# alexkeroro86/SampleNeRFRO

Hardware: AMD Instinct MI355X
Metric: rays/sec (train step) (higher is better)
Workload: dtype f16x3/fp32-acc

## Files before the change

### samplenerfro_amd/csrc/mlp.hip

```cpp
#include "common.h"
#include "nerfmlp_layout.h"
#include "mfma_ops.h"
#include "bkgd_layout.h"
#include "so3_layout.h"

#include <stdlib.h>
#include <type_traits>
#include <vector>
#include <stdio.h>

namespace rnerf {


#define GLOBAL_AS __attribute__((address_space(1)))
#define LDS_AS __attribute__((address_space(3)))

struct MfmaLayer { int dense, ks, nt, kind; };
__host__ __device__ constexpr MfmaLayer mfma_layer(int l) {
  constexpr MfmaLayer t[10] = {{0, 4, 8, 0},  {1, 16, 8, 1}, {2, 16, 8, 1}, {3, 16, 8, 1}, {4, 16, 8, 1},
                               {5, 20, 8, 2}, {6, 16, 8, 1}, {7, 16, 8, 1}, {9, 16, 8, 1}, {10, 18, 4, 3}};
  return t[l];
}
__host__ __device__ constexpr int layer_blocks_before(int l) {
  int o = 0;
// ... 117 lines not shown
    for (int j = 0; j < 8; ++j) {
      const int f = in_feature(l, s, h, j);
      w[j] = f < 0 ? 0.f : params[nerf_koff(d) + f * out_dim + n_out] * PP::WSCALE;
      if constexpr (PP::F16) { if (!(fabsf(w[j]) <= 65504.f)) ((float*)(packed + PP::STREAM_BYTES))[AUX_FLAG] = 1.0f; }
    }
    uint32_t hi[4], lo[4];
    for (int p = 0; p < 4; ++p) split2<F16>(w[2 * p], w[2 * p + 1], hi[p], lo[p]);
    if constexpr (PP::F8X) {
      f8x_mode();
      float wl[8], ws[8];
      for (int p = 0; p < 4; ++p) {
        float ha, hb;
        unpack2<true>(hi[p], ha, hb);
        wl[2 * p] = w[2 * p] - ha; wl[2 * p + 1] = w[2 * p + 1] - hb;
        ws[2 * p] = w[2 * p] * (1.0f / F8X_LO_SCALE); ws[2 * p + 1] = w[2 * p + 1] * (1.0f / F8X_LO_SCALE);
      }
      lo[0] = f8_pair<true>(f8_pair<false>(0u, wl[0], wl[1]), wl[2], wl[3]); lo[1] = f8_pair<true>(f8_pair<false>(0u, wl[4], wl[5]), wl[6], wl[7]);
      lo[2] = f8_pair<true>(f8_pair<false>(0u, ws[0], ws[1]), ws[2], ws[3]); lo[3] = f8_pair<true>(f8_pair<false>(0u, ws[4], ws[5]), ws[6], ws[7]);
    }
    uint4* dst = (uint4*)(packed + (size_t)blk * PP::NP * 1024);
    dst[lane] = make_uint4(hi[0], hi[1], hi[2], hi[3]);
    if constexpr (PP::F8X) { uint2* d2 = (uint2*)(dst + 64); d2[lane] = make_uint2(lo[0], lo[1]); d2[64 + lane] = make_uint2(lo[2], lo[3]); }
    else if (PP::NP == 2) dst[64 + lane] = make_uint4(lo[0], lo[1], lo[2], lo[3]);
  }
  float* aux = (float*)(packed + PP::STREAM_BYTES);
  if (gid < AUX_FLAG) {
    float v = 0.f;
    if (gid < AUX_WSIG) {
      const int l = gid >> 8, n = gid & 255, d = mfma_layer(l).dense;
      v = n < nerf_dense(d).out ? params[nerf_boff(d) + n] : 0.f;
    } else if (gid < AUX_BSIG) v = params[nerf_koff(8) + (gid - AUX_WSIG)];
    else if (gid == AUX_BSIG) v = params[nerf_boff(8)];
    else if (gid >= AUX_WRGB && gid < AUX_BRGB) { const int c = (gid - AUX_WRGB) / 128, n = (gid - AUX_WRGB) % 128; v = params[nerf_koff(11) + n * 3 + c]; }
    else if (gid >= AUX_BRGB && gid < AUX_BRGB + 3) v = params[nerf_boff(11) + (gid - AUX_BRGB)];
    aux[gid] = v;
  }
}

__device__ __forceinline__ void glds16(const char* gsrc, unsigned lds_off) {
  unsigned keep;
  asm volatile("s_mov_b32 %0, m0\n\ts_mov_b32 m0, %2\n\ts_nop 0\n\tglobal_load_lds_dwordx4 %1, off\n\ts_mov_b32 m0, %0"
               : "=&s"(keep) : "v"(gsrc), "s"(lds_off) : "memory");
}
__device__ __forceinline__ void glds16_nt(const char* gsrc, unsigned lds_off) {
  unsigned keep;
  asm volatile("s_mov_b32 %0, m0\n\ts_mov_b32 m0, %2\n\ts_nop 0\n\tglobal_load_lds_dwordx4 %1, off nt\n\ts_mov_b32 m0, %0"
               : "=&s"(keep) : "v"(gsrc), "s"(lds_off) : "memory");
}
__device__ __forceinline__ void glds16_nt_s(const char* sbase, unsigned voff, unsigned lds_off) {
  unsigned keep;
  asm volatile("s_mov_b32 %0, m0\n\ts_mov_b32 m0, %3\n\ts_nop 0\n\tglobal_load_lds_dwordx4 %1, %2 nt\n\ts_mov_b32 m0, %0"
               : "=&s"(keep) : "v"(voff), "s"(sbase), "s"(lds_off) : "memory");
}
__device__ __forceinline__ void slab_wait_dma() { __builtin_amdgcn_s_waitcnt(0x0F70); asm volatile("" ::: "memory"); }

template <int BYTES>
__device__ __forceinline__ void issue_slab(const char* __restrict__ gsrc, unsigned lds_off, int wave, int lane) {
  constexpr int PER_WAVE = BYTES / 4;
  constexpr int N = PER_WAVE / 1024;
  static_assert(N >= 1 && N * 4096 == BYTES, "slab must be a multiple of 4 KiB");
#pragma unroll
  for (int c = 0; c < N; ++c)
    glds16(gsrc + wave * PER_WAVE + c * 1024 + lane * 16,
           __builtin_amdgcn_readfirstlane(lds_off + wave * PER_WAVE + c * 1024));
}

__device__ __forceinline__ uint32_t pk_maxu(uint32_t a, uint32_t b) {
  uint32_t r;
  asm("v_pk_max_u16 %0, %1, %2" : "=v"(r) : "v"(a), "v"(b));
  return r;
}
__device__ __forceinline__ uint32_t pk_min1(uint32_t w) {
  uint32_t r;
  asm("v_pk_min_u16 %0, %1, %2" : "=v"(r) : "v"(w), "v"(0x00010001u));
  return r;
}

typedef float f32x4v __attribute__((ext_vector_type(4)));
__device__ __forceinline__ float4 gload4(const float* p) {
  const f32x4v v = *(const __attribute__((address_space(1))) f32x4v*)p;
  return make_float4(v.x, v.y, v.z, v.w);
}

template <bool ONE_> struct KOpsT { static constexpr bool ONE = ONE_; uint4 h0, l0, h1, l1; };
typedef KOpsT<false> KOps;

constexpr int RELU_FLOOR = 0, NO_FLOOR = (int)0x80000000u;
__device__ __forceinline__ float relu_keep(float x, int floor_bits) {
  const int b = __builtin_bit_cast(int, x);
  return __builtin_bit_cast(float, b > floor_bits ? b : floor_bits);
}

typedef unsigned int u32x4_t __attribute__((ext_vector_type(4)));
__device__ __forceinline__ void stream_store(uint4* p, const uint4 v) {
  u32x4_t t = {v.x, v.y, v.z, v.w};
  __builtin_nontemporal_store(t, (u32x4_t*)p);
}
__device__ __forceinline__ uint4 stream_load(const uint4* p) {
  const u32x4_t t = __builtin_nontemporal_load((const u32x4_t*)p);
  return make_uint4(t.x, t.y, t.z, t.w);
}
typedef unsigned int u32x2_t __attribute__((ext_vector_type(2)));
__device__ __forceinline__ void stream_store8(uint2* p, const uint2 v) {
  u32x2_t t = {v.x, v.y};
  __builtin_nontemporal_store(t, (u32x2_t*)p);
}

// ... 414 lines not shown
      float f[2][8];
#pragma unroll
      for (int mt = 0; mt < (ONE ? 1 : 2); ++mt)
#pragma unroll
        for (int j = 0; j < 8; ++j) {
          const int q = 8 * s + j;
          if (q < nsin) {
            const int d = q / 3, c = q % 3;
            const float x = c == 0 ? v[mt].x : (c == 1 ? v[mt].y : v[mt].z);
            f[mt][j] = pe_sin(fadd(fmul(x, (float)(1 << d)), phase));
          } else if (q == nsin) f[mt][j] = h ? v[mt].z : v[mt].x;
          else if (q == nsin + 1) f[mt][j] = h ? 0.f : v[mt].y;
          else f[mt][j] = 0.f;
        }
      KOps o;
      split8<PREC>(f[0], o.h0, o.l0);
      if constexpr (ONE) { o.h1 = o.h0; o.l1 = o.l0; } else split8<PREC>(f[1], o.h1, o.l1);
      return o;
    };

    auto prev_ops = [&](int s, const float* __restrict__ bias, int floor_v) -> KOps {
      const float4 b0 = *(const float4*)(bias + 16 * s + 4 * h), b1 = *(const float4*)(bias + 16 * s + 8 + 4 * h);
      const float bb[8] = {b0.x, b0.y, b0.z, b0.w, b1.x, b1.y, b1.z, b1.w};
      float r1[8] = {0.f, 0.f, 0.f, 0.f, 0.f, 0.f, 0.f, 0.f};
      if constexpr (!ONE) {
        const float4 u0 = st1[((s >> 1) * 4 + 2 * (s & 1)) * 64], u1 = st1[((s >> 1) * 4 + 2 * (s & 1) + 1) * 64];
        r1[0] = u0.x; r1[1] = u0.y; r1[2] = u0.z; r1[3] = u0.w; r1[4] = u1.x; r1[5] = u1.y; r1[6] = u1.z; r1[7] = u1.w;
      }
      float x0[8], x1[8];
#pragma unroll
      for (int j = 0; j < 8; ++j) {
        x0[j] = relu_keep(fmaf(prev0[s >> 1][8 * (s & 1) + j], INV_SCALE, bb[j]), floor_v);
        x1[j] = relu_keep(fmaf(r1[j], INV_SCALE, bb[j]), floor_v);
      }
      KOps o;
      split8<PREC>(x0, o.h0, o.l0);
      if constexpr (ONE) { o.h1 = o.h0; o.l1 = o.l0; } else split8<PREC>(x1, o.h1, o.l1);
      return o;
    };

    auto load_bias8 = [&](int s, const float* __restrict__ bias, float (&b)[8]) {
      const float4 b0 = *(const float4*)(bias + 16 * s + 4 * h), b1 = *(const float4*)(bias + 16 * s + 8 + 4 * h);
      b[0] = b0.x; b[1] = b0.y; b[2] = b0.z; b[3] = b0.w; b[4] = b1.x; b[5] = b1.y; b[6] = b1.z; b[7] = b1.w;
    };
    auto load_state8 = [&](int s, float (&v)[8]) {
      if constexpr (ONE) return;
      const float4 u0 = st1[((s >> 1) * 4 + 2 * (s & 1)) * 64], u1 = st1[((s >> 1) * 4 + 2 * (s & 1) + 1) * 64];
      v[0] = u0.x; v[1] = u0.y; v[2] = u0.z; v[3] = u0.w; v[4] = u1.x; v[5] = u1.y; v[6] = u1.z; v[7] = u1.w;
    };
    NoWork nowork;

#define SLAB_PREFETCH(DO_NEXT)                                                                                       \
  do { if (DO_NEXT) { issue_slab<SLAB>(packed + off, (unsigned)((buf ^ 1) * SLAB), wave, lane); off += SLAB; } } while (0)
#define SLAB_DONE() do { slab_wait_dma(); __syncthreads(); buf ^= 1; } while (0)

    float sig0 = 0.f, sig1 = 0.f;

    KOps cur;
    {
      cur = enc_ops(pd, 0, 30);
      SeamWork<PREC, TRAIN != 0, ONE> seam(acc0, acc1, prev0, st1);
      seam.cv.floor_v = RELU_FLOOR;
      load_bias8(0, auxt + AUX_BIAS, seam.cv.b);
      load_bias8(0, auxt + AUX_ZERO, seam.cv.ws);
#define RNERF_PE_KSTEP(S, FIRST_, SAVE_)                                                                             \
      {                                                                                                              \
        if (SAVE_) save_ops(SAVE_PE + S, cur);                                                                       \
        watch(cur, true);          \
        SLAB_PREFETCH(true);    \
        if constexpr (S < 3) {                                                                                       \
          EncWork<PREC, S + 1, 30, ONE> ew(pd, h);                                                                        \
          kstep_mfma<PREC, 8, 0, FIRST_>(acc0, acc1, cur, smem + buf * SLAB, lane, ew);                              \
          cur = ew.result();                                                                                         \
        } else {                                                                                                     \
          kstep_mfma<PREC, 8, 0, false>(acc0, acc1, cur, smem + buf * SLAB, lane, seam);                             \
        }                                                                                                            \
        SLAB_DONE();                                                                                                 \
      }
      RNERF_PE_KSTEP(0, true, true) RNERF_PE_KSTEP(1, false, true) RNERF_PE_KSTEP(2, false, true) RNERF_PE_KSTEP(3, false, true)
      seam.finish();
      cur = seam.cv.result();
    }

    float bnext[8], wnext[8];
    load_bias8(1, auxt + AUX_BIAS, bnext);
    load_bias8(1, auxt + AUX_ZERO, wnext);

#pragma unroll 1
    for (int l = 1; l <= 8; ++l) {
      const float* __restrict__ bias = auxt + AUX_BIAS + 256 * (l - 1);
      SeamWork<PREC, TRAIN != 0, ONE> seam(acc0, acc1, prev0, st1);
      seam.cv.floor_v = l == 8 ? NO_FLOOR : RELU_FLOOR;
      const float* __restrict__ wseam = auxt + (l == 7 ? AUX_WSIG : AUX_ZERO);
      const float* __restrict__ wsel = auxt + (l == 8 ? AUX_WSIG : AUX_ZERO);
#define RNERF_KSTEP(S)                                                                                              \
      {                                                                                                              \
        save_ops(SAVE_L1 + 16 * (l - 1) + S, cur);                                                                   \
        watch(cur, false);                                                                                           \
        if constexpr (TRAIN != 0 && S == 0) save_mask(l - 1, 0, nz_nibbles(cur.h0), nz_nibbles(cur.h1));                  \
        if constexpr (S == 13) { load_bias8(0, bias + 256, seam.cv.b); load_bias8(0, wseam, seam.cv.ws); }           \
        float bnn[8], wnn[8];                                                                                        \
        if constexpr (S + 2 < 16) { load_bias8(S + 2, bias, bnn); load_bias8(S + 2, wsel, wnn); }    \
        else if constexpr (S == 14) { load_bias8(1, bias + 256, bnn); load_bias8(1, wseam, wnn); }    \
        auto dma = [&]() { SLAB_PREFETCH(true); };                                                                   \
        if constexpr (S + 1 < 16) {                                                                                  \
          PrevConv<PREC, S + 1, TRAIN != 0, true, ONE> cv(prev0[(S + 1) >> 1]);                                           \
          cv.floor_v = RELU_FLOOR;                                                                                        \
          _Pragma("unroll") for (int j = 0; j < 8; ++j) { cv.b[j] = bnext[j]; cv.ws[j] = wnext[j]; }                 \
          load_state8(S + 1, cv.v1);                                                                                 \
          kstep_mfma<PREC, 8, 0, S == 0, PrevConv<PREC, S + 1, TRAIN != 0, true, ONE>, decltype(dma)>(acc0, acc1, cur, smem + buf * SLAB, lane, cv, dma); \
          cur = cv.result();                                                                                         \
          sig0 += cv.sg0; sig1 += cv.sg1;                                                                            \
          save_mask(l - 1, S + 1, cv.nz[0], cv.nz[1]);                                                               \
        } else {                                                                                                     \
           \
           \
          kstep_mfma<PREC, 8, 0, false, SeamWork<PREC, TRAIN != 0, ONE>, decltype(dma)>(acc0, acc1, cur, smem + buf * SLAB, lane, seam, dma); \
        }                                                                                                            \
        if constexpr (S + 2 <= 16) { _Pragma("unroll") for (int j = 0; j < 8; ++j) { bnext[j] = bnn[j]; wnext[j] = wnn[j]; } } \
        SLAB_DONE();                                                                                                 \
      }
      RNERF_KSTEP(0) RNERF_KSTEP(1) RNERF_KSTEP(2) RNERF_KSTEP(3) RNERF_KSTEP(4) RNERF_KSTEP(5) RNERF_KSTEP(6) RNERF_KSTEP(7)
      RNERF_KSTEP(8) RNERF_KSTEP(9) RNERF_KSTEP(10) RNERF_KSTEP(11) RNERF_KSTEP(12) RNERF_KSTEP(13) RNERF_KSTEP(14) RNERF_KSTEP(15)
#undef RNERF_KSTEP
      if (l == 5) {
        asm volatile("" : "+v"(pd[0].x), "+v"(pd[0].y), "+v"(pd[0].z), "+v"(pd[1].x), "+v"(pd[1].y), "+v"(pd[1].z));
        cur = enc_ops(pd, 0, 30);
        RNERF_PE_KSTEP(0, false, false) RNERF_PE_KSTEP(1, false, false) RNERF_PE_KSTEP(2, false, false) RNERF_PE_KSTEP(3, false, false)
      }
      seam.finish();
      cur = seam.cv.result();
      sig0 += seam.cv.sg0; sig1 += seam.cv.sg1;
    }

    {
      const float* __restrict__ bias = auxt + AUX_BIAS + 256 * 8;
      KOps c0 = cur;
      KOps c1 = prev_ops(1, bias, NO_FLOOR);
      float bA[8], bB[8];
      load_bias8(2, bias, bA);
      load_bias8(3, bias, bB);
#define RNERF_VSLAB(SL)                                                                                              \
      {                                                                                                              \
        save_ops(SAVE_L1 + 16 * 8 + 2 * SL, c0);                                                                     \
        save_ops(SAVE_L1 + 16 * 8 + 2 * SL + 1, c1);                                                                 \
        watch(c0, true); watch(c1, true);                                                                            \
        SLAB_PREFETCH(true);                                                                                         \
        if constexpr (SL + 1 < 8) {                                                                                  \
          float bA2[8], bB2[8];                                                                                      \
          if constexpr (SL + 2 < 8) { load_bias8(2 * SL + 4, bias, bA2); load_bias8(2 * SL + 5, bias, bB2); }        \
          PrevConv<PREC, 2 * SL + 2, false, false, ONE> cvA(prev0[SL + 1]);                                                      \
          PrevConv<PREC, 2 * SL + 3, false, false, ONE> cvB(prev0[SL + 1]);                                                      \
          cvA.floor_v = NO_FLOOR; cvB.floor_v = NO_FLOOR;                                                                \
          _Pragma("unroll") for (int j = 0; j < 8; ++j) { cvA.b[j] = bA[j]; cvB.b[j] = bB[j]; }                      \
          load_state8(2 * SL + 2, cvA.v1);                                                                           \
          load_state8(2 * SL + 3, cvB.v1);                                                                           \
          PairOfPairs<decltype(cvA)> wA(cvA);                                                                        \
          PairOfPairs<decltype(cvB)> wB(cvB);                                                                        \
          kstep_mfma<PREC, 4, 0, SL == 0>(acc0, acc1, c0, smem + buf * SLAB, lane, wA);                              \
          kstep_mfma<PREC, 4, 1, false>(acc0, acc1, c1, smem + buf * SLAB, lane, wB);                                \
          c0 = cvA.result(); c1 = cvB.result();                                                                      \
          if constexpr (SL + 2 < 8) { _Pragma("unroll") for (int j = 0; j < 8; ++j) { bA[j] = bA2[j]; bB[j] = bB2[j]; } } \
        } else {                                                                                                     \
          const KOps n0 = enc_ops(dr, 0, 12), n1 = enc_ops(dr, 1, 12);                                               \
          kstep_mfma<PREC, 4, 0, false>(acc0, acc1, c0, smem + buf * SLAB, lane, nowork);                            \
          kstep_mfma<PREC, 4, 1, false>(acc0, acc1, c1, smem + buf * SLAB, lane, nowork);                            \
          c0 = n0; c1 = n1;                                                                                          \
        }                                                                                                            \
        SLAB_DONE();                                                                                                 \
      }
      RNERF_VSLAB(0) RNERF_VSLAB(1) RNERF_VSLAB(2) RNERF_VSLAB(3) RNERF_VSLAB(4) RNERF_VSLAB(5) RNERF_VSLAB(6) RNERF_VSLAB(7)
#undef RNERF_VSLAB
      save_ops(SAVE_VIEW, c0);
      save_ops(SAVE_VIEW + 1, c1);
      watch(c0, true); watch(c1, true);
      next_tile = tileq != nullptr ? __builtin_amdgcn_readfirstlane(__hip_atomic_load(tileq + 1 + blockIdx.x, __ATOMIC_RELAXED, __HIP_MEMORY_SCOPE_AGENT))
                                   : find_next(tile + (int)gridDim.x);
      const bool has_next_tile = next_tile < n_tiles;
      if (has_next_tile) off = 0;
      SLAB_PREFETCH(has_next_tile);
      kstep_mfma<PREC, 4, 0, false>(acc0, acc1, c0, smem + buf * SLAB, lane, nowork);
      kstep_mfma<PREC, 4, 1, false>(acc0, acc1, c1, smem + buf * SLAB, lane, nowork);
      SLAB_DONE();
    }

    {
      const float* __restrict__ hw = auxt + 4 * h;
      auto head_load = [&](int t, float4 (&W)[16]) {
#pragma unroll
        for (int g = 0; g < 4; ++g) {
          const int n = 32 * t + 8 * g;
          W[4 * g] = gload4(hw + AUX_BIAS + 256 * 9 + n);
          W[4 * g + 1] = gload4(hw + AUX_WRGB + n); W[4 * g + 2] = gload4(hw + AUX_WRGB + 128 + n); W[4 * g + 3] = gload4(hw + AUX_WRGB + 256 + n);
        }
      };
      float p0[3] = {0.f, 0.f, 0.f}, p1[3] = {0.f, 0.f, 0.f};
      float4 Wc[16];
      head_load(0, Wc);
#pragma unroll
      for (int t = 0; t < 4; ++t) {
        float4 Wn[16];
        if (t + 1 < 4) head_load(t + 1, Wn);
        RNERF_PIN();
        float rv0[16], rv1[16];
#pragma unroll
        for (int g = 0; g < 4; ++g) {
          const float4 bb = Wc[4 * g], wr = Wc[4 * g + 1], wg = Wc[4 * g + 2], wb = Wc[4 * g + 3];
          const float bv[4] = {bb.x, bb.y, bb.z, bb.w}, wrv[4] = {wr.x, wr.y, wr.z, wr.w}, wgv[4] = {wg.x, wg.y, wg.z, wg.w}, wbv[4] = {wb.x, wb.y, wb.z, wb.w};
#pragma unroll
          for (int i = 0; i < 4; ++i) {
            const float v0 = relu_keep(fmaf(acc0[t][4 * g + i], INV_SCALE, bv[i]), RELU_FLOOR);
            p0[0] = fmaf(v0, wrv[i], p0[0]); p0[1] = fmaf(v0, wgv[i], p0[1]); p0[2] = fmaf(v0, wbv[i], p0[2]);
            rv0[4 * g + i] = v0;
            if constexpr (!ONE) {
              const float v1 = relu_keep(fmaf(acc1[t][4 * g + i], INV_SCALE, bv[i]), RELU_FLOOR);
              p1[0] = fmaf(v1, wrv[i], p1[0]); p1[1] = fmaf(v1, wgv[i], p1[1]); p1[2] = fmaf(v1, wbv[i], p1[2]);
              rv1[4 * g + i] = v1;
            } else rv1[4 * g + i] = v0;
          }
        }
        if (t + 1 < 4) {
#pragma unroll
          for (int q = 0; q < 16; ++q) Wc[q] = Wn[q];
        }
        if constexpr (TRAIN != 0) {
#pragma unroll
          for (int half = 0; half < 2; ++half) {
            KOps o;
            float a0[8], a1[8];
#pragma unroll
            for (int j = 0; j < 8; ++j) { a0[j] = rv0[8 * half + j]; a1[j] = rv1[8 * half + j]; }
            if constexpr (TRAIN >= 2) { split8<PREC>(a0, o.h0, o.l0); split8<PREC>(a1, o.h1, o.l1); }
            else {
              o.h0 = make_uint4(pack2<PP::F16>(a0[0], a0[1]), pack2<PP::F16>(a0[2], a0[3]), pack2<PP::F16>(a0[4], a0[5]), pack2<PP::F16>(a0[6], a0[7]));
              o.h1 = make_uint4(pack2<PP::F16>(a1[0], a1[1]), pack2<PP::F16>(a1[2], a1[3]), pack2<PP::F16>(a1[4], a1[5]), pack2<PP::F16>(a1[6], a1[7]));
            }
// ... 20 lines not shown
      }
      if constexpr (PP::F16 && !PP::F8X) {
        if (auxt[AUX_FLAG] != 0.f) { const float qn = __builtin_nanf(""); p0[0] = p0[1] = p0[2] = qn; p1[0] = p1[1] = p1[2] = qn; sig0 = qn; sig1 = qn; }
      }
      if (h == 0) {
        if constexpr (REDO) {
          if (row_ok[0] && __builtin_isnan(out_raw[row[0]].x)) out_raw[row[0]] = make_float4(p0[0], p0[1], p0[2], sig0);
          if (row_ok[1] && __builtin_isnan(out_raw[row[1]].x)) out_raw[row[1]] = make_float4(p1[0], p1[1], p1[2], sig1);
        } else {
          if (row_ok[0]) out_raw[row[0]] = make_float4(p0[0], p0[1], p0[2], sig0);
          if (row_ok[1]) out_raw[row[1]] = make_float4(p1[0], p1[1], p1[2], sig1);
        }
      }
    }
#undef RNERF_PE_KSTEP
#undef SLAB_PREFETCH
#undef SLAB_DONE
    tile = next_tile;
  }
}

constexpr int DY_L9 = 144, DY_HEADS = 152, DY_SLOTS = 153;
constexpr int DGRAD_PASSES = 22;
constexpr int kBwdF16OnePass = 3;
constexpr int kBwdBlocks = 8 * 8 + 8 * 16 * 8;

__host__ __device__ constexpr int bwd_dense(int i) { return i == 0 ? 10 : (i == 1 ? 9 : 9 - i); }
__host__ __device__ constexpr int bwd_blocks_before(int i) { return i == 0 ? 0 : 64 + (i - 1) * 128; }

template <int PREC>
__global__ void nerfmlp_pack_bwd_kernel(const float* __restrict__ params, char* __restrict__ packed) {
  using PP = Prec<PREC>;
  const int gid = blockIdx.x * blockDim.x + threadIdx.x;
  if (gid >= kBwdBlocks * 64) return;
  const int blk = gid >> 6, lane = gid & 63;
  int i = 0;
  while (i < 8 && blk >= bwd_blocks_before(i + 1)) ++i;
  const int rel = blk - bwd_blocks_before(i);
  const int s = rel / 8, kt = rel % 8;
  const int d = bwd_dense(i), out_dim = nerf_dense(d).out;
  const int kf = 32 * kt + (lane & 31), h = lane >> 5;
  float w[8];
  for (int j = 0; j < 8; ++j) {
    const int n = prev_feature(s, h, j);
    w[j] = n < out_dim ? params[nerf_koff(d) + kf * out_dim + n] * PP::WSCALE : 0.f;
  }
  uint32_t hi[4], lo[4];
  for (int p = 0; p < 4; ++p) split2<PP::F16>(w[2 * p], w[2 * p + 1], hi[p], lo[p]);
  uint4* dst = (uint4*)(packed + (size_t)blk * PP::NP * 1024);
  dst[lane] = make_uint4(hi[0], hi[1], hi[2], hi[3]);
  if (PP::NP == 2) dst[64 + lane] = make_uint4(lo[0], lo[1], lo[2], lo[3]);
}

template <int PREC, int S, bool NEED_LO, bool ONE = false>
struct GradConv {
  using PP = Prec<PREC>;
  const f32x16& p0;
  float v1[8];
  float t0[8], t1[8];
  uint32_t w0, w1;
  uint32_t hi[2][4], lo[2][4];
  float x0, x1;
  __device__ __forceinline__ GradConv(const f32x16& p) : p0(p) {}
  template <int C, int PI>
  __device__ __forceinline__ void chunk() {
    constexpr int mt = PI >> 2, p = PI & 3;
    if constexpr (ONE && mt == 1) return;
    constexpr float INV_SCALE = 1.0f / PP::WSCALE;
    if constexpr (C == 0) {
      const float r0 = mt == 0 ? p0[8 * (S & 1) + 2 * p] : v1[2 * p];
      const float r1 = mt == 0 ? p0[8 * (S & 1) + 2 * p + 1] : v1[2 * p + 1];
      x0 = fmaf(r0, INV_SCALE, mt == 0 ? t0[2 * p] : t1[2 * p]);
      x1 = fmaf(r1, INV_SCALE, mt == 0 ? t0[2 * p + 1] : t1[2 * p + 1]);
    } else if constexpr (C == 1) {
      const uint32_t w = mt == 0 ? w0 : w1;
      constexpr int pos0 = 8 * (S & 3) + p, pos1 = pos0 + 4;
      uint32_t m0, m1;
      asm("v_bfe_i32 %0, %1, %2, 1" : "=v"(m0) : "v"(w), "n"(pos0));
      asm("v_bfe_i32 %0, %1, %2, 1" : "=v"(m1) : "v"(w), "n"(pos1));
      x0 = __builtin_bit_cast(float, __builtin_bit_cast(uint32_t, x0) & m0);
      x1 = __builtin_bit_cast(float, __builtin_bit_cast(uint32_t, x1) & m1);
    } else if constexpr (C == 2) {
      hi[mt][p] = pack2<PP::F16>(x0, x1);
    } else if constexpr (C == 3) {
      if constexpr (NEED_LO) {
        float ha, hb;
        unpack2<PP::F16>(hi[mt][p], ha, hb);
        x0 -= ha; x1 -= hb;
      }
    } else {
      if constexpr (NEED_LO) lo[mt][p] = pack2<PP::F16>(x0, x1);
      else lo[mt][p] = 0;
    }
  }
  __device__ __forceinline__ KOpsT<ONE> result() const {
    KOpsT<ONE> o;
    o.h0 = make_uint4(hi[0][0], hi[0][1], hi[0][2], hi[0][3]); o.l0 = make_uint4(lo[0][0], lo[0][1], lo[0][2], lo[0][3]);
    if constexpr (ONE) { o.h1 = o.h0; o.l1 = o.l0; }
    else { o.h1 = make_uint4(hi[1][0], hi[1][1], hi[1][2], hi[1][3]); o.l1 = make_uint4(lo[1][0], lo[1][1], lo[1][2], lo[1][3]); }
    return o;
  }
};

template <int BWD> struct Bwd {
  static constexpr bool F16 = BWD != RNERF_BWD_BF16;
  static constexpr bool LO8 = BWD == RNERF_BWD_F16X3_LO8;
  static constexpr int NP = (BWD == RNERF_BWD_F16X2 || LO8) ? 2 : 1;
  static constexpr int PREC = F16 ? RNERF_PREC_F16X3 : RNERF_PREC_BF16X3;
  static constexpr int PASSES = (BWD == RNERF_BWD_F16X2 || LO8) ? 3 : (BWD == RNERF_BWD_F16 ? 22 : (BWD == kBwdF16OnePass ? 1 : DGRAD_PASSES));
  static constexpr bool NEED_LO = PASSES != 22 && PASSES != 1;
};
__host__ __device__ constexpr size_t dy_plane_uint4(long long R, int np) { return (size_t)DY_SLOTS * np * (size_t)R * 2; }
__host__ __device__ constexpr size_t dy_addr(int q, long long t32, int m, int h) { return (((size_t)t32 * DY_SLOTS + q) * 32 + m) * 2 + h; }

template <int BWD, bool ONE = false>
__global__ void __launch_bounds__(256, 1)
nerfmlp_dgrad_kernel(const char* __restrict__ packed_bwd, const float* __restrict__ fwd_aux, const uint4* __restrict__ saved,
                     long long save_rows, const float4* __restrict__ d_raw, long long total_rows, int n_tiles,
                     uint4* __restrict__ dy) {
  using BW = Bwd<BWD>;
  using KOps = KOpsT<ONE>;
  constexpr int PREC = BW::PREC;
  constexpr int DGP = BW::PASSES;
  constexpr bool NEED_LO = BW::NEED_LO;
  using PP = Prec<PREC>;
  constexpr int SLAB = PP::SLAB;
// ... 53 lines not shown
    };
    auto mask_at = [&](int set, uint4& a, uint4& b) {
      const uint32_t* src = (const uint32_t*)(saved + sv_mask0(save_rows)) + sv_mask_addr(set * 4, t32_0, m, h);
      constexpr size_t ws = 64, mt1 = 36 * 64;
#define RNERF_NTL(P) __builtin_nontemporal_load(P)
      a = make_uint4(RNERF_NTL(src), RNERF_NTL(src + ws), RNERF_NTL(src + 2 * ws), RNERF_NTL(src + 3 * ws));
      if constexpr (ONE) b = make_uint4(0, 0, 0, 0);
      else b = make_uint4(RNERF_NTL(src + mt1), RNERF_NTL(src + ws + mt1), RNERF_NTL(src + 2 * ws + mt1), RNERF_NTL(src + 3 * ws + mt1));
#undef RNERF_NTL
    };
    auto grad_ops = [&](int s, bool use_mask, const uint4 mk0, const uint4 mk1, const float* __restrict__ wadd) -> KOps {
      float r1[8] = {0.f, 0.f, 0.f, 0.f, 0.f, 0.f, 0.f, 0.f};
      if constexpr (!ONE) {
        const float4 u0 = st1[((s >> 1) * 4 + 2 * (s & 1)) * 64], u1 = st1[((s >> 1) * 4 + 2 * (s & 1) + 1) * 64];
        r1[0] = u0.x; r1[1] = u0.y; r1[2] = u0.z; r1[3] = u0.w; r1[4] = u1.x; r1[5] = u1.y; r1[6] = u1.z; r1[7] = u1.w;
      }
      const uint32_t w0 = (s >> 2) == 0 ? mk0.x : ((s >> 2) == 1 ? mk0.y : ((s >> 2) == 2 ? mk0.z : mk0.w));
      const uint32_t w1 = (s >> 2) == 0 ? mk1.x : ((s >> 2) == 1 ? mk1.y : ((s >> 2) == 2 ? mk1.z : mk1.w));
      float x0[8], x1[8];
#pragma unroll
      for (int j = 0; j < 8; ++j) {
        float a = prev0[s >> 1][8 * (s & 1) + j] * INV_SCALE, b = r1[j] * INV_SCALE;
        if (wadd) { const float w = wadd[16 * s + 8 * (j >> 2) + 4 * h + (j & 3)]; a = fmaf(g[0].w, w, a); b = fmaf(g[1].w, w, b); }
        if (use_mask) {
          const uint32_t bit = 1u << (8 * (s & 3) + (j >> 1) + 4 * (j & 1));
          a = (w0 & bit) ? a : 0.f;
          b = (w1 & bit) ? b : 0.f;
        }
        x0[j] = a; x1[j] = b;
      }
      KOps o;
      if constexpr (ONE) { split8<PREC>(x0, o.h0, o.l0); if constexpr (!(NEED_LO || BW::NP == 2)) o.l0 = make_uint4(0, 0, 0, 0); o.h1 = o.h0; o.l1 = o.l0; }
      else if constexpr (NEED_LO || BW::NP == 2) { split8<PREC>(x0, o.h0, o.l0); split8<PREC>(x1, o.h1, o.l1); }
      else {
        o.h0 = make_uint4(pack2<PP::F16>(x0[0], x0[1]), pack2<PP::F16>(x0[2], x0[3]), pack2<PP::F16>(x0[4], x0[5]), pack2<PP::F16>(x0[6], x0[7]));
        o.h1 = make_uint4(pack2<PP::F16>(x1[0], x1[1]), pack2<PP::F16>(x1[2], x1[3]), pack2<PP::F16>(x1[4], x1[5]), pack2<PP::F16>(x1[6], x1[7]));
        o.l0 = make_uint4(0, 0, 0, 0); o.l1 = o.l0;
      }
      return o;
    };
    auto layer_end = [&]() {
#pragma unroll
      for (int t = 0; t < 8; ++t) {
        prev0[t] = acc0[t];
        if constexpr (!ONE) {
#pragma unroll
          for (int rq = 0; rq < 4; ++rq)
            st1[(t * 4 + rq) * 64] = make_float4(acc1[t][4 * rq], acc1[t][4 * rq + 1], acc1[t][4 * rq + 2], acc1[t][4 * rq + 3]);
        }
      }
    };
#define SLAB_PREFETCH(DO_NEXT)                                                                                       \
  do { if (DO_NEXT) { issue_slab<SLAB>(packed_bwd + off, (unsigned)((buf ^ 1) * SLAB), wave, lane); off += SLAB; } } while (0)
#define SLAB_DONE() do { slab_wait_dma(); __syncthreads(); buf ^= 1; } while (0)

    {
      KOps o;
      float hz0[8] = {0, 0, 0, 0, 0, 0, 0, 0}, hz1[8] = {0, 0, 0, 0, 0, 0, 0, 0};
      if (h == 0) { hz0[0] = g[0].w; hz0[1] = g[0].x; hz0[2] = g[0].y; hz0[3] = g[0].z; hz1[0] = g[1].w; hz1[1] = g[1].x; hz1[2] = g[1].y; hz1[3] = g[1].z; }
      split8<PREC>(hz0, o.h0, o.l0);
      if constexpr (ONE) { o.h1 = o.h0; o.l1 = o.l0; } else split8<PREC>(hz1, o.h1, o.l1);
      dy_store(DY_HEADS, o);
#pragma unroll
      for (int t = 0; t < 8; ++t)
#pragma unroll
        for (int r = 0; r < 16; ++r) {
          float a = 0.f, b = 0.f;
          if (t < 4) {
            const int n = 32 * t + (r & 3) + 8 * (r >> 2) + 4 * h;
            const float wr = fwd_aux[AUX_WRGB + n], wg = fwd_aux[AUX_WRGB + 128 + n], wb = fwd_aux[AUX_WRGB + 256 + n];
            a = (g[0].x * wr + g[0].y * wg + g[0].z * wb) * PP::WSCALE;
            b = (g[1].x * wr + g[1].y * wg + g[1].z * wb) * PP::WSCALE;
          }
          acc0[t][r] = a;
          if constexpr (!ONE) acc1[t][r] = b;
        }
      layer_end();
    }

    {
      uint4 ma, mb;
      mask_at(8, ma, mb);
      KOps cur = grad_ops(0, true, ma, mb, nullptr);
#define RNERF_DG_KSTEP(S, NSTEPS, SLOT0, PREFETCH_STMT)                                                                       \
      {                                                                                                                         \
        dy_store((SLOT0) + S, cur);                                                                                             \
        auto dma = [&]() { PREFETCH_STMT; };    \
        if constexpr (S + 1 < NSTEPS) {                                                                                         \
          GradConv<PREC, S + 1, NEED_LO, ONE> cv(prev0[(S + 1) >> 1]);                                                                   \
          if constexpr (!ONE) {                                                                                                 \
            const float4 u0 = st1[(((S + 1) >> 1) * 4 + 2 * ((S + 1) & 1)) * 64], u1 = st1[(((S + 1) >> 1) * 4 + 2 * ((S + 1) & 1) + 1) * 64]; \
            cv.v1[0] = u0.x; cv.v1[1] = u0.y; cv.v1[2] = u0.z; cv.v1[3] = u0.w; cv.v1[4] = u1.x; cv.v1[5] = u1.y; cv.v1[6] = u1.z; cv.v1[7] = u1.w; \
          }                                                                                                                     \
          if (wadd) {            \
            const float4 wa = *(const float4*)(wadd + 16 * (S + 1) + 4 * h), wb = *(const float4*)(wadd + 16 * (S + 1) + 8 + 4 * h); \
            const float wv[8] = {wa.x, wa.y, wa.z, wa.w, wb.x, wb.y, wb.z, wb.w};                                               \
            _Pragma("unroll") for (int j = 0; j < 8; ++j) { cv.t0[j] = g[0].w * wv[j]; cv.t1[j] = g[1].w * wv[j]; }             \
          } else {                                                                                                              \
            _Pragma("unroll") for (int j = 0; j < 8; ++j) { cv.t0[j] = 0.f; cv.t1[j] = 0.f; }                                   \
          }                                                                                                                     \
          cv.w0 = ((S + 1) >> 2) == 0 ? ma.x : (((S + 1) >> 2) == 1 ? ma.y : (((S + 1) >> 2) == 2 ? ma.z : ma.w));             \
          cv.w1 = ((S + 1) >> 2) == 0 ? mb.x : (((S + 1) >> 2) == 1 ? mb.y : (((S + 1) >> 2) == 2 ? mb.z : mb.w));             \
          kstep_mfma<PREC, 8, 0, S == 0, GradConv<PREC, S + 1, NEED_LO, ONE>, decltype(dma), DGP>(acc0, acc1, cur, smem + buf * SLAB, lane, cv, dma); \
          cur = cv.result();                                                                                                    \
        } else {                                                                                                                \
          kstep_mfma<PREC, 8, 0, false, NoWork, decltype(dma), DGP>(acc0, acc1, cur, smem + buf * SLAB, lane, nowork, dma);         \
        }                                                                                                                       \
        SLAB_DONE();                                                                                                            \
      }
      {
        const float* __restrict__ wadd = nullptr;
        RNERF_DG_KSTEP(0, 8, DY_L9, SLAB_PREFETCH(true)) RNERF_DG_KSTEP(1, 8, DY_L9, SLAB_PREFETCH(true))
        RNERF_DG_KSTEP(2, 8, DY_L9, SLAB_PREFETCH(true)) RNERF_DG_KSTEP(3, 8, DY_L9, SLAB_PREFETCH(true))
        RNERF_DG_KSTEP(4, 8, DY_L9, SLAB_PREFETCH(true)) RNERF_DG_KSTEP(5, 8, DY_L9, SLAB_PREFETCH(true))
        RNERF_DG_KSTEP(6, 8, DY_L9, SLAB_PREFETCH(true)) RNERF_DG_KSTEP(7, 8, DY_L9, SLAB_PREFETCH(true))
      }
      layer_end();
    }

    uint4 nma = make_uint4(0, 0, 0, 0), nmb = nma;
#pragma unroll 1
    for (int l = 8; l >= 1; --l) {
      const bool use_mask = l != 8;
      const float* __restrict__ wadd = (l == 7) ? fwd_aux + AUX_WSIG : nullptr;
      uint4 ma = nma, mb = nmb;
      if (!use_mask) { ma = make_uint4(~0u, ~0u, ~0u, ~0u); mb = ma; }
      mask_at(l - 1, nma, nmb);
      KOps cur = grad_ops(0, true, ma, mb, wadd);
      const int slot0 = 16 * l;
#define RNERF_DG_PF(S) do { if ((S) == 15 && l == 1) { if (has_next_tile) off = 0; SLAB_PREFETCH(has_next_tile); } else SLAB_PREFETCH(true); } while (0)
      RNERF_DG_KSTEP(0, 16, slot0, RNERF_DG_PF(0)) RNERF_DG_KSTEP(1, 16, slot0, RNERF_DG_PF(1)) RNERF_DG_KSTEP(2, 16, slot0, RNERF_DG_PF(2))
      RNERF_DG_KSTEP(3, 16, slot0, RNERF_DG_PF(3)) RNERF_DG_KSTEP(4, 16, slot0, RNERF_DG_PF(4)) RNERF_DG_KSTEP(5, 16, slot0, RNERF_DG_PF(5))
      RNERF_DG_KSTEP(6, 16, slot0, RNERF_DG_PF(6)) RNERF_DG_KSTEP(7, 16, slot0, RNERF_DG_PF(7)) RNERF_DG_KSTEP(8, 16, slot0, RNERF_DG_PF(8))
      RNERF_DG_KSTEP(9, 16, slot0, RNERF_DG_PF(9)) RNERF_DG_KSTEP(10, 16, slot0, RNERF_DG_PF(10)) RNERF_DG_KSTEP(11, 16, slot0, RNERF_DG_PF(11))
      RNERF_DG_KSTEP(12, 16, slot0, RNERF_DG_PF(12)) RNERF_DG_KSTEP(13, 16, slot0, RNERF_DG_PF(13)) RNERF_DG_KSTEP(14, 16, slot0, RNERF_DG_PF(14))
      RNERF_DG_KSTEP(15, 16, slot0, RNERF_DG_PF(15))
#undef RNERF_DG_PF
      layer_end();
    }
#undef RNERF_DG_KSTEP

#pragma unroll
    for (int s = 0; s < 16; ++s) {
      const KOps o = grad_ops(s, true, nma, nmb, nullptr);
      dy_store(s, o);
    }
#undef SLAB_PREFETCH
#undef SLAB_DONE
  }
  if constexpr (BW::F16) {
#pragma unroll
    for (int o = 32; o >= 1; o >>= 1) mref = fmaxf(mref, __shfl_xor(mref, o));
    if (lane == 0 && mref > 0.f)
      atomicMax((unsigned int*)((float*)(dy + dy_plane_uint4(save_rows, BW::NP)) + save_rows), __builtin_bit_cast(unsigned int, mref));
  }
}

template <bool F16>
__device__ __forceinline__ uint4 shifted_identity(int lane, int a) {
  const int col = lane & 31, h = lane >> 5;
  uint32_t w[4] = {0, 0, 0, 0};
  if ((col >> 4) == a && ((col >> 3) & 1) == h) { const int j = col & 7; w[j >> 1] = (F16 ? 0x3C00u : 0x3F80u) << (16 * (j & 1)); }
  return make_uint4(w[0], w[1], w[2], w[3]);
}

__device__ __forceinline__ void pack_rows_bf16(const f32x16& d, uint4& u0, uint4& u1) {
  u0 = make_uint4(pack2<false>(d[0], d[1]), pack2<false>(d[2], d[3]), pack2<false>(d[4], d[5]), pack2<false>(d[6], d[7]));
  u1 = make_uint4(pack2<false>(d[8], d[9]), pack2<false>(d[10], d[11]), pack2<false>(d[12], d[13]), pack2<false>(d[14], d[15]));
}

struct WgradJob {
  int dense;
  int xkind;
  int row_off;
  int dkind;
  int KT, NT, write_bias;
  int KTa, xkind2, row_off2, NTa, dense2, dkind2;
// ... 1875 lines not shown
```

Before: 670,800.

## Use counted vmcnt waits and move activation saves behind slab prefetch

Replaces the full vmcnt(0) wait plus __syncthreads at each slab boundary with a counted wait that lets the activation saves, mask saves and dy stores still be in flight, followed by an lgkm wait and a raw s_barrier. Those global stores are moved after the slab DMA issue (inside the dma lambda), so the counted wait covers only the slab loads. In the backward pass, the per-step wadd weight loads are software-pipelined two steps ahead through a templated GradConv, and loads against the zero auxiliary buffer stand in for the runtime branch. The aim is to stop the store traffic from stalling the double-buffered weight pipeline. The cost is correctness that depends on exact vmcnt accounting.

```diff
diff --git a/samplenerfro_amd/csrc/mlp.hip b/samplenerfro_amd/csrc/mlp.hip
--- a/samplenerfro_amd/csrc/mlp.hip
+++ b/samplenerfro_amd/csrc/mlp.hip
@@ -193,7 +193,26 @@
   asm volatile("s_mov_b32 %0, m0\n\ts_mov_b32 m0, %3\n\ts_nop 0\n\tglobal_load_lds_dwordx4 %1, %2 nt\n\ts_mov_b32 m0, %0"
                : "=&s"(keep) : "v"(voff), "s"(sbase), "s"(lds_off) : "memory");
 }
-__device__ __forceinline__ void slab_wait_dma() { __builtin_amdgcn_s_waitcnt(0x0F70); asm volatile("" ::: "memory"); }
+template <int YOUNGER = 0>
+__device__ __forceinline__ void slab_wait_dma() {
+  static_assert(YOUNGER >= 0 && YOUNGER < 64, "vmcnt is a 6-bit field on gfx9");
+  __builtin_amdgcn_s_waitcnt(0x0F70 | (YOUNGER & 15) | ((YOUNGER >> 4) << 14));
+  asm volatile("" ::: "memory");
+}
+
+template <bool COUNTED, int YOUNGER>
+__device__ __forceinline__ void slab_done_sync() {
+  if constexpr (COUNTED) {
+    slab_wait_dma<YOUNGER>();
+    __builtin_amdgcn_s_waitcnt(0xC07F);
+    asm volatile("" ::: "memory");
+    __builtin_amdgcn_s_barrier();
+    asm volatile("" ::: "memory");
+  } else {
+    slab_wait_dma<0>();
+    __syncthreads();
+  }
+}
 
 template <int BYTES>
 __device__ __forceinline__ void issue_slab(const char* __restrict__ gsrc, unsigned lds_off, int wave, int lane) {
@@ -714,7 +733,8 @@
 
 #define SLAB_PREFETCH(DO_NEXT)                                                                                       \
   do { if (DO_NEXT) { issue_slab<SLAB>(packed + off, (unsigned)((buf ^ 1) * SLAB), wave, lane); off += SLAB; } } while (0)
-#define SLAB_DONE() do { slab_wait_dma(); __syncthreads(); buf ^= 1; } while (0)
+#define SLAB_DONE(YOUNGER) do { slab_done_sync<TRAIN != 0, (TRAIN != 0 ? (YOUNGER) : 0)>(); buf ^= 1; } while (0)
+    constexpr int SAVE_VM = TRAIN == 0 ? 0 : (TRAIN == 1 ? 1 : 2) * (ONE ? 1 : 2), MASK_VM = TRAIN == 0 ? 0 : (ONE ? 1 : 2);
 
     float sig0 = 0.f, sig1 = 0.f;
 
@@ -727,9 +747,9 @@
       load_bias8(0, auxt + AUX_ZERO, seam.cv.ws);
 #define RNERF_PE_KSTEP(S, FIRST_, SAVE_)                                                                             \
       {                                                                                                              \
-        if (SAVE_) save_ops(SAVE_PE + S, cur);                                                                       \
         watch(cur, true);          \
         SLAB_PREFETCH(true);    \
+        if (SAVE_) save_ops(SAVE_PE + S, cur);             \
         if constexpr (S < 3) {                                                                                       \
           EncWork<PREC, S + 1, 30, ONE> ew(pd, h);                                                                        \
           kstep_mfma<PREC, 8, 0, FIRST_>(acc0, acc1, cur, smem + buf * SLAB, lane, ew);                              \
@@ -737,7 +757,7 @@
         } else {                                                                                                     \
           kstep_mfma<PREC, 8, 0, false>(acc0, acc1, cur, smem + buf * SLAB, lane, seam);                             \
         }                                                                                                            \
-        SLAB_DONE();                                                                                                 \
+        SLAB_DONE((SAVE_) ? SAVE_VM : 0);                                                                            \
       }
       RNERF_PE_KSTEP(0, true, true) RNERF_PE_KSTEP(1, false, true) RNERF_PE_KSTEP(2, false, true) RNERF_PE_KSTEP(3, false, true)
       seam.finish();
@@ -757,14 +777,15 @@
       const float* __restrict__ wsel = auxt + (l == 8 ? AUX_WSIG : AUX_ZERO);
 #define RNERF_KSTEP(S)                                                                                              \
       {                                                                                                              \
-        save_ops(SAVE_L1 + 16 * (l - 1) + S, cur);                                                                   \
         watch(cur, false);                                                                                           \
         if constexpr (TRAIN != 0 && S == 0) save_mask(l - 1, 0, nz_nibbles(cur.h0), nz_nibbles(cur.h1));                  \
         if constexpr (S == 13) { load_bias8(0, bias + 256, seam.cv.b); load_bias8(0, wseam, seam.cv.ws); }           \
         float bnn[8], wnn[8];                                                                                        \
         if constexpr (S + 2 < 16) { load_bias8(S + 2, bias, bnn); load_bias8(S + 2, wsel, wnn); }    \
         else if constexpr (S == 14) { load_bias8(1, bias + 256, bnn); load_bias8(1, wseam, wnn); }    \
-        auto dma = [&]() { SLAB_PREFETCH(true); };                                                                   \
+         \
+                 \
+        auto dma = [&]() { SLAB_PREFETCH(true); save_ops(SAVE_L1 + 16 * (l - 1) + S, cur); };                        \
         if constexpr (S + 1 < 16) {                                                                                  \
           PrevConv<PREC, S + 1, TRAIN != 0, true, ONE> cv(prev0[(S + 1) >> 1]);                                           \
           cv.floor_v = RELU_FLOOR;                                                                                        \
@@ -780,7 +801,7 @@
           kstep_mfma<PREC, 8, 0, false, SeamWork<PREC, TRAIN != 0, ONE>, decltype(dma)>(acc0, acc1, cur, smem + buf * SLAB, lane, seam, dma); \
         }                                                                                                            \
         if constexpr (S + 2 <= 16) { _Pragma("unroll") for (int j = 0; j < 8; ++j) { bnext[j] = bnn[j]; wnext[j] = wnn[j]; } } \
-        SLAB_DONE();                                                                                                 \
+        SLAB_DONE(SAVE_VM + ((S + 1 < 16 && ((S + 1) & 3) == 3) ? MASK_VM : 0));    \
       }
       RNERF_KSTEP(0) RNERF_KSTEP(1) RNERF_KSTEP(2) RNERF_KSTEP(3) RNERF_KSTEP(4) RNERF_KSTEP(5) RNERF_KSTEP(6) RNERF_KSTEP(7)
       RNERF_KSTEP(8) RNERF_KSTEP(9) RNERF_KSTEP(10) RNERF_KSTEP(11) RNERF_KSTEP(12) RNERF_KSTEP(13) RNERF_KSTEP(14) RNERF_KSTEP(15)
@@ -804,13 +825,15 @@
       load_bias8(3, bias, bB);
 #define RNERF_VSLAB(SL)                                                                                              \
       {                                                                                                              \
+        watch(c0, true); watch(c1, true);                                                                            \
+        float bA2[8], bB2[8];                                                                                        \
+        auto vbias = [&]() { if constexpr (SL + 2 < 8) { load_bias8(2 * SL + 4, bias, bA2); load_bias8(2 * SL + 5, bias, bB2); } }; \
+        if constexpr (TRAIN != 0) vbias();       \
+        SLAB_PREFETCH(true);                                                                                         \
         save_ops(SAVE_L1 + 16 * 8 + 2 * SL, c0);                                                                     \
         save_ops(SAVE_L1 + 16 * 8 + 2 * SL + 1, c1);                                                                 \
-        watch(c0, true); watch(c1, true);                                                                            \
-        SLAB_PREFETCH(true);                                                                                         \
+        if constexpr (TRAIN == 0) vbias();       \
         if constexpr (SL + 1 < 8) {                                                                                  \
-          float bA2[8], bB2[8];                                                                                      \
-          if constexpr (SL + 2 < 8) { load_bias8(2 * SL + 4, bias, bA2); load_bias8(2 * SL + 5, bias, bB2); }        \
           PrevConv<PREC, 2 * SL + 2, false, false, ONE> cvA(prev0[SL + 1]);                                                      \
           PrevConv<PREC, 2 * SL + 3, false, false, ONE> cvB(prev0[SL + 1]);                                                      \
           cvA.floor_v = NO_FLOOR; cvB.floor_v = NO_FLOOR;                                                                \
@@ -829,21 +852,21 @@
           kstep_mfma<PREC, 4, 1, false>(acc0, acc1, c1, smem + buf * SLAB, lane, nowork);                            \
           c0 = n0; c1 = n1;                                                                                          \
         }                                                                                                            \
-        SLAB_DONE();                                                                                                 \
+        SLAB_DONE(2 * SAVE_VM);                                                                                      \
       }
       RNERF_VSLAB(0) RNERF_VSLAB(1) RNERF_VSLAB(2) RNERF_VSLAB(3) RNERF_VSLAB(4) RNERF_VSLAB(5) RNERF_VSLAB(6) RNERF_VSLAB(7)
 #undef RNERF_VSLAB
-      save_ops(SAVE_VIEW, c0);
-      save_ops(SAVE_VIEW + 1, c1);
       watch(c0, true); watch(c1, true);
       next_tile = tileq != nullptr ? __builtin_amdgcn_readfirstlane(__hip_atomic_load(tileq + 1 + blockIdx.x, __ATOMIC_RELAXED, __HIP_MEMORY_SCOPE_AGENT))
                                    : find_next(tile + (int)gridDim.x);
       const bool has_next_tile = next_tile < n_tiles;
       if (has_next_tile) off = 0;
       SLAB_PREFETCH(has_next_tile);
+      save_ops(SAVE_VIEW, c0);
+      save_ops(SAVE_VIEW + 1, c1);
       kstep_mfma<PREC, 4, 0, false>(acc0, acc1, c0, smem + buf * SLAB, lane, nowork);
       kstep_mfma<PREC, 4, 1, false>(acc0, acc1, c1, smem + buf * SLAB, lane, nowork);
-      SLAB_DONE();
+      SLAB_DONE(2 * SAVE_VM);
     }
 
     {
@@ -970,12 +993,13 @@
   if (PP::NP == 2) dst[64 + lane] = make_uint4(lo[0], lo[1], lo[2], lo[3]);
 }
 
-template <int PREC, int S, bool NEED_LO, bool ONE = false>
+template <int PREC, int S, bool NEED_LO, bool ONE = false, bool WADD = false>
 struct GradConv {
   using PP = Prec<PREC>;
   const f32x16& p0;
   float v1[8];
-  float t0[8], t1[8];
+  float wv[8];
+  float gs0, gs1;
   uint32_t w0, w1;
   uint32_t hi[2][4], lo[2][4];
   float x0, x1;
@@ -988,8 +1012,10 @@
     if constexpr (C == 0) {
       const float r0 = mt == 0 ? p0[8 * (S & 1) + 2 * p] : v1[2 * p];
       const float r1 = mt == 0 ? p0[8 * (S & 1) + 2 * p + 1] : v1[2 * p + 1];
-      x0 = fmaf(r0, INV_SCALE, mt == 0 ? t0[2 * p] : t1[2 * p]);
-      x1 = fmaf(r1, INV_SCALE, mt == 0 ? t0[2 * p + 1] : t1[2 * p + 1]);
+      float ta = 0.f, tb = 0.f;
+      if constexpr (WADD) { ta = fmul(mt == 0 ? gs0 : gs1, wv[2 * p]); tb = fmul(mt == 0 ? gs0 : gs1, wv[2 * p + 1]); }
+      x0 = fmaf(r0, INV_SCALE, ta);
+      x1 = fmaf(r1, INV_SCALE, tb);
     } else if constexpr (C == 1) {
       const uint32_t w = mt == 0 ? w0 : w1;
       constexpr int pos0 = 8 * (S & 3) + p, pos1 = pos0 + 4;
@@ -1149,7 +1175,12 @@
     };
 #define SLAB_PREFETCH(DO_NEXT)                                                                                       \
   do { if (DO_NEXT) { issue_slab<SLAB>(packed_bwd + off, (unsigned)((buf ^ 1) * SLAB), wave, lane); off += SLAB; } } while (0)
-#define SLAB_DONE() do { slab_wait_dma(); __syncthreads(); buf ^= 1; } while (0)
+    constexpr int DY_VM = (ONE ? 1 : 2) * BW::NP;
+#define SLAB_DONE() do { slab_done_sync<true, DY_VM>(); buf ^= 1; } while (0)
+    auto load_w8 = [&](int s, const float* __restrict__ wsrc, float (&w)[8]) {
+      const float4 a = gload4(wsrc + 16 * s + 4 * h), b = gload4(wsrc + 16 * s + 8 + 4 * h);
+      w[0] = a.x; w[1] = a.y; w[2] = a.z; w[3] = a.w; w[4] = b.x; w[5] = b.y; w[6] = b.z; w[7] = b.w;
+    };
 
     {
       KOps o;
@@ -1181,32 +1212,36 @@
       KOps cur = grad_ops(0, true, ma, mb, nullptr);
 #define RNERF_DG_KSTEP(S, NSTEPS, SLOT0, PREFETCH_STMT)                                                                       \
       {                                                                                                                         \
-        dy_store((SLOT0) + S, cur);                                                                                             \
-        auto dma = [&]() { PREFETCH_STMT; };    \
+        float wnn[8];                                                                                                           \
+        if constexpr (kWadd && S + 2 < NSTEPS) load_w8(S + 2, wsrc, wnn);                       \
+         \
+         \
+        auto dma = [&]() { PREFETCH_STMT; dy_store((SLOT0) + S, cur); };                                                        \
         if constexpr (S + 1 < NSTEPS) {                                                                                         \
-          GradConv<PREC, S + 1, NEED_LO, ONE> cv(prev0[(S + 1) >> 1]);                                                                   \
+          GradConv<PREC, S + 1, NEED_LO, ONE, kWadd> cv(prev0[(S + 1) >> 1]);                                                   \
           if constexpr (!ONE) {                                                                                                 \
             const float4 u0 = st1[(((S + 1) >> 1) * 4 + 2 * ((S + 1) & 1)) * 64], u1 = st1[(((S + 1) >> 1) * 4 + 2 * ((S + 1) & 1) + 1) * 64]; \
             cv.v1[0] = u0.x; cv.v1[1] = u0.y; cv.v1[2] = u0.z; cv.v1[3] = u0.w; cv.v1[4] = u1.x; cv.v1[5] = u1.y; cv.v1[6] = u1.z; cv.v1[7] = u1.w; \
           }                                                                                                                     \
-          if (wadd) {            \
-            const float4 wa = *(const float4*)(wadd + 16 * (S + 1) + 4 * h), wb = *(const float4*)(wadd + 16 * (S + 1) + 8 + 4 * h); \
-            const float wv[8] = {wa.x, wa.y, wa.z, wa.w, wb.x, wb.y, wb.z, wb.w};                                               \
-            _Pragma("unroll") for (int j = 0; j < 8; ++j) { cv.t0[j] = g[0].w * wv[j]; cv.t1[j] = g[1].w * wv[j]; }             \
-          } else {                                                                                                              \
-            _Pragma("unroll") for (int j = 0; j < 8; ++j) { cv.t0[j] = 0.f; cv.t1[j] = 0.f; }                                   \
+          if constexpr (kWadd) {                                                                                                \
+            _Pragma("unroll") for (int j = 0; j < 8; ++j) cv.wv[j] = wnext[j];                                                  \
+            cv.gs0 = gs0; cv.gs1 = gs1;                                                                                         \
           }                                                                                                                     \
           cv.w0 = ((S + 1) >> 2) == 0 ? ma.x : (((S + 1) >> 2) == 1 ? ma.y : (((S + 1) >> 2) == 2 ? ma.z : ma.w));             \
           cv.w1 = ((S + 1) >> 2) == 0 ? mb.x : (((S + 1) >> 2) == 1 ? mb.y : (((S + 1) >> 2) == 2 ? mb.z : mb.w));             \
-          kstep_mfma<PREC, 8, 0, S == 0, GradConv<PREC, S + 1, NEED_LO, ONE>, decltype(dma), DGP>(acc0, acc1, cur, smem + buf * SLAB, lane, cv, dma); \
+          kstep_mfma<PREC, 8, 0, S == 0, GradConv<PREC, S + 1, NEED_LO, ONE, kWadd>, decltype(dma), DGP>(acc0, acc1, cur, smem + buf * SLAB, lane, cv, dma); \
           cur = cv.result();                                                                                                    \
         } else {                                                                                                                \
           kstep_mfma<PREC, 8, 0, false, NoWork, decltype(dma), DGP>(acc0, acc1, cur, smem + buf * SLAB, lane, nowork, dma);         \
         }                                                                                                                       \
+        if constexpr (kWadd && S + 2 < NSTEPS) { _Pragma("unroll") for (int j = 0; j < 8; ++j) wnext[j] = wnn[j]; }             \
         SLAB_DONE();                                                                                                            \
       }
       {
-        const float* __restrict__ wadd = nullptr;
+        constexpr bool kWadd = false;
+        const float* __restrict__ wsrc = nullptr;
+        float wnext[8] = {0.f, 0.f, 0.f, 0.f, 0.f, 0.f, 0.f, 0.f};
+        const float gs0 = 0.f, gs1 = 0.f;
         RNERF_DG_KSTEP(0, 8, DY_L9, SLAB_PREFETCH(true)) RNERF_DG_KSTEP(1, 8, DY_L9, SLAB_PREFETCH(true))
         RNERF_DG_KSTEP(2, 8, DY_L9, SLAB_PREFETCH(true)) RNERF_DG_KSTEP(3, 8, DY_L9, SLAB_PREFETCH(true))
         RNERF_DG_KSTEP(4, 8, DY_L9, SLAB_PREFETCH(true)) RNERF_DG_KSTEP(5, 8, DY_L9, SLAB_PREFETCH(true))
@@ -1220,6 +1255,11 @@
     for (int l = 8; l >= 1; --l) {
       const bool use_mask = l != 8;
       const float* __restrict__ wadd = (l == 7) ? fwd_aux + AUX_WSIG : nullptr;
+      constexpr bool kWadd = true;
+      const float* __restrict__ wsrc = fwd_aux + (l == 7 ? AUX_WSIG : AUX_ZERO);
+      const float gs0 = l == 7 ? g[0].w : 0.f, gs1 = l == 7 ? g[1].w : 0.f;
+      float wnext[8];
+      load_w8(1, wsrc, wnext);
       uint4 ma = nma, mb = nmb;
       if (!use_mask) { ma = make_uint4(~0u, ~0u, ~0u, ~0u); mb = ma; }
       mask_at(l - 1, nma, nmb);
```

Result: no change. 673,800 (median of 6 runs) (+0.4%).
